# LinXueyuanStdio/LaTeX_OCR

Measured on NVIDIA H100. Metric: formula-images/sec (train step, 128x512 px, seq<=150), higher is better.
Workload: dtype bf16

## Files before the change

latex_ocr_b200/csrc/lo_common.cuh:

```cuda
#pragma once
#include <cuda_runtime.h>
#include <cuda_bf16.h>
#include <stdint.h>
#include <stdio.h>
#include <string.h>

#include "../../include/latex_ocr_b200.h"

typedef __nv_bfloat16 bf16;

namespace lo {

extern char g_err[512];
extern int64_t g_launches;

inline int fail(int code, const char* fmt, const char* a = "", long b = 0, long c = 0) {
  snprintf(g_err, sizeof(g_err), fmt, a, b, c);
  return code;
}

#define LO_CHECK_ARG(cond, what)                                                        \
  do {                                                                                  \
    if (!(cond)) return lo::fail(LO_EINVAL, "%s: invalid argument: " what " (line %ld)", __func__, __LINE__); \
  } while (0)

#define LO_CUDA(call)                                                                   \
  do {                                                                                  \
    cudaError_t e__ = (call);                                                           \
    if (e__ != cudaSuccess)                                                             \
      return lo::fail(LO_ECUDA, "%s: CUDA error %ld at line %ld", cudaGetErrorString(e__), (long)e__, __LINE__); \
  } while (0)

#define LO_LAUNCH_OK()                                                                  \
  do {                                                                                  \
    lo::g_launches++;                                                                   \
    cudaError_t e__ = cudaGetLastError();                                               \
    if (e__ != cudaSuccess)                                                             \
      return lo::fail(LO_ECUDA, "%s: launch failed (%ld) at line %ld", cudaGetErrorString(e__), (long)e__, __LINE__); \
  } while (0)

#define LO_TRY(call)                                                                    \
  do {                                                                                  \
    int r__ = (call);                                                                   \
    if (r__ != LO_OK) return r__;                                                       \
  } while (0)

inline int cdiv(long a, long b) { return (int)((a + b - 1) / b); }

constexpr int LO_NUM_SMS = 132;

#define LO_OPTIONS(X)                                                                                           \
  X(g_opt_att_pipe, "att_pipe", 1)                 \
  X(g_opt_pdl, "pdl", 1)                                                   \
  X(g_opt_att_abi_pdl, "att_abi_pdl", 0)             \
  X(g_opt_att_l2_keep_mb, "att_l2_keep_mb", 24)    \
  X(g_opt_att_nsplit, "att_nsplit", 0)                       \
  X(g_opt_att_cluster, "att_cluster", 1)                      \
  X(g_opt_att_maskbits, "att_maskbits", 1)                 \
  X(g_opt_att_bwd_mma, "att_bwd_mma", 1)                     \
  X(g_opt_dec_streams, "dec_streams", 1)             \
  X(g_opt_dec_fuse, "dec_fuse", 0)                                        \
  X(g_opt_dec_fuse_bwd, "dec_fuse_bwd", 0)                               \
  X(g_opt_dec_cl, "dec_cl", 0)                                                 \
  X(g_opt_dec_cl_bwd, "dec_cl_bwd", 0)                                        \
  X(g_opt_fuse_lstm, "fuse_lstm", 0)                               \
  X(g_opt_skinny_mma, "skinny_mma", 1)                               \
  X(g_opt_skinny_tma, "skinny_tma", 1)                                    \
  X(g_opt_skinny8, "skinny8", 1)                                        \
  X(g_opt_conv_persist, "conv_persist", 1)                      \
  X(g_opt_conv_mt2, "conv_mt2", 1)                            \
  X(g_opt_conv_mc, "conv_mc", 1)                                     \
  X(g_opt_wgrad256, "wgrad256", 0)                                   \
  X(g_opt_det, "deterministic", 0)                                             \
  X(g_opt_dbg_skip, "dbg_skip", 0)                                  \
  X(g_opt_l2_persist_mb, "l2_persist_mb", 0)

#define LO_OPTION_EXTERN(var, name, def) extern int var;
LO_OPTIONS(LO_OPTION_EXTERN)
#undef LO_OPTION_EXTERN

template <typename... KArgs, typename... Args>
inline cudaError_t launch_pdl(void (*kernel)(KArgs...), dim3 grid, dim3 block, size_t smem, cudaStream_t st, Args... args) {
  cudaLaunchConfig_t cfg{};
  cfg.gridDim = grid;
  cfg.blockDim = block;
  cfg.dynamicSmemBytes = smem;
  cfg.stream = st;
  cudaLaunchAttribute attr[1];
  attr[0].id = cudaLaunchAttributeProgrammaticStreamSerialization;
  attr[0].val.programmaticStreamSerializationAllowed = 1;
  cfg.attrs = attr;
  cfg.numAttrs = g_opt_pdl ? 1 : 0;
  return cudaLaunchKernelEx(&cfg, kernel, KArgs(args)...);
}
template <typename... KArgs, typename... Args>
inline cudaError_t launch_cluster(void (*kernel)(KArgs...), dim3 grid, dim3 block, size_t smem, cudaStream_t st, dim3 cl, bool pdl,
                                  Args... args) {
  cudaLaunchConfig_t cfg{};
  cfg.gridDim = grid;
  cfg.blockDim = block;
  cfg.dynamicSmemBytes = smem;
  cfg.stream = st;
  cudaLaunchAttribute attr[2];
  int n = 0;
  attr[n].id = cudaLaunchAttributeClusterDimension;
  attr[n].val.clusterDim.x = cl.x;
  attr[n].val.clusterDim.y = cl.y;
  attr[n].val.clusterDim.z = cl.z;
  n++;
  if (pdl && g_opt_pdl) {
    attr[n].id = cudaLaunchAttributeProgrammaticStreamSerialization;
    attr[n].val.programmaticStreamSerializationAllowed = 1;
    n++;
  }
  cfg.attrs = attr;
  cfg.numAttrs = n;
  return cudaLaunchKernelEx(&cfg, kernel, KArgs(args)...);
}

__device__ __forceinline__ float ldf(const float* p) { return *p; }
__device__ __forceinline__ float ldf(const bf16* p) { return __bfloat162float(*p); }
__device__ __forceinline__ void stf(float* p, float v) { *p = v; }
__device__ __forceinline__ void stf(bf16* p, float v) { *p = __float2bfloat16_rn(v); }
__device__ __forceinline__ float roundto(float v, const float*) { return v; }
__device__ __forceinline__ float roundto(float v, const bf16*) { return __bfloat162float(__float2bfloat16_rn(v)); }

__device__ __forceinline__ void ld8(const float* p, float* v) {
  float4 a = *reinterpret_cast<const float4*>(p);
  float4 b = *reinterpret_cast<const float4*>(p + 4);
  v[0] = a.x; v[1] = a.y; v[2] = a.z; v[3] = a.w; v[4] = b.x; v[5] = b.y; v[6] = b.z; v[7] = b.w;
}
__device__ __forceinline__ void ld8(const bf16* p, float* v) {
  uint4 u = *reinterpret_cast<const uint4*>(p);
  const uint32_t w[4] = {u.x, u.y, u.z, u.w};
#pragma unroll
  for (int i = 0; i < 4; i++) {
    v[2 * i] = __uint_as_float(w[i] << 16);
    v[2 * i + 1] = __uint_as_float(w[i] & 0xffff0000u);
  }
}
__device__ __forceinline__ void lds8(uint32_t saddr, float* v, const float*) {
  float4 a, b;
  asm volatile("ld.shared.v4.f32 {%0, %1, %2, %3}, [%4];" : "=f"(a.x), "=f"(a.y), "=f"(a.z), "=f"(a.w) : "r"(saddr));
  asm volatile("ld.shared.v4.f32 {%0, %1, %2, %3}, [%4];" : "=f"(b.x), "=f"(b.y), "=f"(b.z), "=f"(b.w) : "r"(saddr + 16));
  v[0] = a.x; v[1] = a.y; v[2] = a.z; v[3] = a.w; v[4] = b.x; v[5] = b.y; v[6] = b.z; v[7] = b.w;
}
__device__ __forceinline__ void lds8(uint32_t saddr, float* v, const bf16*) {
  uint32_t w[4];
  asm volatile("ld.shared.v4.b32 {%0, %1, %2, %3}, [%4];" : "=r"(w[0]), "=r"(w[1]), "=r"(w[2]), "=r"(w[3]) : "r"(saddr));
#pragma unroll
  for (int i = 0; i < 4; i++) {
    v[2 * i] = __uint_as_float(w[i] << 16);
    v[2 * i + 1] = __uint_as_float(w[i] & 0xffff0000u);
  }
}
__device__ __forceinline__ void st8(float* p, const float* v) {
  *reinterpret_cast<float4*>(p) = make_float4(v[0], v[1], v[2], v[3]);
  *reinterpret_cast<float4*>(p + 4) = make_float4(v[4], v[5], v[6], v[7]);
}
__device__ __forceinline__ void st8(bf16* p, const float* v) {
  uint32_t w[4];
#pragma unroll
  for (int i = 0; i < 4; i++) {
    __nv_bfloat162 h = __floats2bfloat162_rn(v[2 * i], v[2 * i + 1]);
    w[i] = *reinterpret_cast<uint32_t*>(&h);
  }
  *reinterpret_cast<uint4*>(p) = make_uint4(w[0], w[1], w[2], w[3]);
}

__device__ __forceinline__ float warp_sum(float v) {
#pragma unroll
  for (int o = 16; o > 0; o >>= 1) v += __shfl_xor_sync(0xffffffffu, v, o);
  return v;
}
__device__ __forceinline__ float warp_max(float v) {
#pragma unroll
  for (int o = 16; o > 0; o >>= 1) v = fmaxf(v, __shfl_xor_sync(0xffffffffu, v, o));
  return v;
}
__device__ __forceinline__ float sigmoidf_(float x) { return 1.0f / (1.0f + expf(-x)); }

__device__ __forceinline__ uint4 philox4x32_10(uint4 c, uint2 k) {
#pragma unroll
  for (int r = 0; r < 10; r++) {
    const uint32_t hi0 = __umulhi(0xD2511F53u, c.x), lo0 = 0xD2511F53u * c.x;
    const uint32_t hi1 = __umulhi(0xCD9E8D57u, c.z), lo1 = 0xCD9E8D57u * c.z;
    c = make_uint4(hi1 ^ c.y ^ k.x, lo1, hi0 ^ c.w ^ k.y, lo0);
    k.x += 0x9E3779B9u;
    k.y += 0xBB67AE85u;
  }
  return c;
}
__device__ __forceinline__ float u01(uint32_t x) { return (float)(x >> 8) * (1.0f / 16777216.0f); }
__device__ __forceinline__ float philox_dropout_mult(const unsigned long long* state, int b, int t, int j, float p, float scale) {
  const unsigned long long seed = state[0], call = state[1];
  const uint4 r = philox4x32_10(make_uint4((uint32_t)(j >> 2), (uint32_t)t, (uint32_t)b, (uint32_t)call),
                                make_uint2((uint32_t)seed, (uint32_t)(seed >> 32)));
  const uint32_t w = (j & 3) == 0 ? r.x : ((j & 3) == 1 ? r.y : ((j & 3) == 2 ? r.z : r.w));
  return u01(w) >= p ? scale : 0.f;
}

#define LO_DISPATCH_DT(dt, T, ...)                   \
  do {                                               \
    if ((dt) == LO_F32) { typedef float T; __VA_ARGS__; } \
    else if ((dt) == LO_BF16) { typedef bf16 T; __VA_ARGS__; } \
    else return lo::fail(LO_EINVAL, "%s: bad dtype %ld", __func__, (long)(dt)); \
  } while (0)

struct GemmDesc {
  int M, N, K;
  int64_t sam, sak, sbk, sbn, ldc;
  int batch;
  int64_t sA, sB, sC;
  const float* bias;
  int accumulate, relu;
};
int gemm(const void* A, int dtA, const void* B, int dtB, void* C, int dtC, const GemmDesc& d, int impl, cudaStream_t st);
int gemm_nt(const void* A, int dtA, int64_t lda, const void* W, int dtW, int64_t ldw, void* C, int dtC, int64_t ldc,
            int M, int N, int K, const float* bias, int accumulate, int relu, int impl, cudaStream_t st);
int gemm_tn(const void* A, int dtA, int64_t lda, const void* B, int dtB, int64_t ldb, void* C, int dtC, int64_t ldc,
            int M, int N, int K, int accumulate, int impl, cudaStream_t st);
int gemm_nn(const void* A, int dtA, int64_t lda, const void* B, int dtB, int64_t ldb, void* C, int dtC, int64_t ldc,
            int M, int N, int K, int accumulate, int impl, cudaStream_t st);
int colsum(const void* X, int dt, float* out, int M, int N, int64_t ld, int accumulate, cudaStream_t st);

struct AttFwdArgs {
  const void *att1, *enc;
  const float* att2; int64_t att2_stride;
  const float* wf;
  float* alpha; int64_t alpha_stride;
  float* ctx; float* gate_pre; int64_t gate_stride; float* gctx; bf16* gctx_bf;
  int B, R;
  void* work;
  int rows_per_img;
  int nsplit_hint;
  int act;
  int a_ch;
  uint8_t* mask_out;
  int abi = 0;
};
struct AttBwdArgs {
  const void *att1, *enc;
  const float *att2, *gate; int64_t o1_stride;
  const float* wf; const float* alpha; int64_t alpha_stride;
  const float* ctx; const float* dgctx; int64_t dg_stride;
  const float* dreg; int64_t dreg_stride; const float* sreg; int64_t sreg_stride;
  float* de; float* datt2; float* dgp; int64_t dcat_stride; bf16* datt2_bf; bf16* dgp_bf; float* dctx_out;
  int B, R;
  void* work;
  float* dwf_part;
  int nsplit_hint;
  int act;
  int a_ch;
  const uint8_t* mask_in;
  int abi = 0;
  void* datt1 = nullptr;
  int ordered_dwf = 0;
};
int attention_fwd_pipe(const AttFwdArgs& x, int dt, int C, cudaStream_t st);
int attention_bwd_pipe(const AttBwdArgs& x, int dt, int C, cudaStream_t st);
inline int64_t att_partials_offset(int B) { return B <= 1024 ? 4096 : ((int64_t)B * 4 + 255) / 256 * 256; }
struct AttRagged {
  const int32_t* reg_off;
  const int32_t* reg_off_host;
  void* map;
  int ctas;
};
int64_t attention_ragged_map_bytes(int B);
int attention_ragged_prepare(AttRagged& rg, int B, int rpi, cudaStream_t st);
int attention_fwd_ragged(const AttFwdArgs& x, const AttRagged& rg, int dt, int C, cudaStream_t st);

bool tc_available();
int tc_gemm_nt(const bf16* A, int64_t lda, const bf16* W, int64_t ldw, void* C, int dtC, int64_t ldc,
               int M, int N, int K, const float* bias, int accumulate, int relu, cudaStream_t st);
int tc_gemm_nt_ex(const bf16* A, int64_t lda, const bf16* W, int64_t ldw, void* C, int dtC, int64_t ldc, int M, int N, int K,
                  const float* bias, int accumulate, int relu, int splits, int atomic_acc, int small_n_tile, cudaStream_t st);
struct TcLstmEpi {
  const float* ptab; const int64_t* tok; int64_t tok_stride;
  const float* hh; int64_t hh_stride;
  const float* c_prev; float* gates; float* c_out; float* h_out; bf16* h_bf;
  float* hd; int64_t hd_stride; const float* dmask;
  int D, V;
  const unsigned long long* dstate; float dp; int row0, t_idx;
};
struct DecStepFwd {
  const bf16* gctx; int64_t ld_gctx;
  const bf16* wil; int64_t ld_wil;
  TcLstmEpi e;
  const bf16* wcat; int64_t ld_wcat;
  const float* bcat; float* o1_next; int64_t ld_o1; int N2;
  unsigned int* bar; unsigned int bar_target;
  int M, K;
};
int dec_step_fwd(const DecStepFwd& p, cudaStream_t st);
struct DecStepBwd {
  const bf16* dcat_a; int64_t ld_dcat;
  const bf16* wbwd2; int64_t ld_w2; int K2;
  int Ma;
  const float* dhd; int64_t dhd_stride; const float* dmask; const unsigned long long* dstate; float dp; int t_idx;
  float* dc; const float* gates; const float* c_prev; const float* c_cur;
  float* dG; bf16* dG_bf; int64_t dG_stride;
  const bf16* wbwd1; int64_t ld_w1; int K1;
  int Mb;
  float* dxh; int C, D;
  unsigned int* bar; unsigned int bar_target;
};
int dec_step_bwd(const DecStepBwd& p, cudaStream_t st);
bool dec_cl_fwd_ok(int D, int C, int N2);
bool dec_cl_bwd_ok(int D, int C, int A);
int dec_cl_fwd(const DecStepFwd& p, cudaStream_t st);
int dec_cl_bwd(const DecStepBwd& p, cudaStream_t st);
int cl_set_ts(long long* p);
int sk_set_ts(long long* p);
int tc_gemm_nt_lstm(const bf16* A, int64_t lda, const bf16* Wil, int64_t ldw, int M, int D, int K, const TcLstmEpi& e, cudaStream_t st);
int skinny_gemm_nt_lstm(const bf16* A, int64_t lda, const bf16* Wil, int64_t ldw, int M, int D, int K, const TcLstmEpi& e, cudaStream_t st);
int skinny_gemm_nt(const bf16* A, int64_t lda, const bf16* W, int64_t ldw, float* C, int64_t ldc, int M, int N, int K, const float* bias,
                   int splits, int atomic_acc, cudaStream_t st);
int tc_gemm_tn(const bf16* A, int64_t lda, const bf16* B, int64_t ldb, float* C, int64_t ldc, int M, int N, int K, cudaStream_t st);
int tc_gemm_tn_batched(const bf16* A, int64_t sAk, int64_t sAb, const bf16* B, int64_t sBk, int64_t sBb, float* C, int64_t ldc,
                       int64_t sCb, int M, int N, int K, int batch, cudaStream_t st);
int tc_conv3x3_wgrad(const bf16* x, const bf16* dy, float* dw, int N, int H, int W, int Cin, int Cout, int pad, cudaStream_t st);
int tc_conv3x3(const bf16* x, const bf16* w, const float* bias, const bf16* mask, bf16* y,
               int N, int H, int W, int Cin, int Cout, int pad, int relu, cudaStream_t st);

}
```

latex_ocr_b200/csrc/lo_tc.cu:

```cuda
#include <cuda.h>

#include <mutex>
#include <unordered_map>

#include "lo_common.cuh"
#include "lo_ptx.cuh"
#include "lo_wgmma.cuh"

namespace lo {

__device__ __forceinline__ void tma_load_2d(void* dst, const CUtensorMap* map, uint64_t* bar, int c0, int c1) {
  asm volatile("cp.async.bulk.tensor.2d.shared::cluster.global.mbarrier::complete_tx::bytes [%0], [%1, {%3, %4}], [%2];" ::"r"(
                   smem_u32(dst)),
               "l"(reinterpret_cast<uint64_t>(map)), "r"(smem_u32(bar)), "r"(c0), "r"(c1)
               : "memory");
}
__device__ __forceinline__ void tma_load_2d_hint(void* dst, const CUtensorMap* map, uint64_t* bar, int c0, int c1, uint64_t policy) {
  asm volatile(
      "cp.async.bulk.tensor.2d.shared::cluster.global.mbarrier::complete_tx::bytes.L2::cache_hint [%0], [%1, {%3, %4}], [%2], %5;" ::"r"(
          smem_u32(dst)),
      "l"(reinterpret_cast<uint64_t>(map)), "r"(smem_u32(bar)), "r"(c0), "r"(c1), "l"(policy)
      : "memory");
}
__device__ __forceinline__ void tma_load_3d(void* dst, const CUtensorMap* map, uint64_t* bar, int c0, int c1, int c2) {
// ... 286 lines not shown
          tc_store_pair(p, row_off + n0 + c, acc[4 * i + 2 * h] + s_bias[c], acc[4 * i + 2 * h + 1] + s_bias[c + 1], use_mask);
        }
      }
    }
    if (dbg && threadIdx.x == 0) p.dbg[6] = clock64();
  }
  if (MC) cluster_sync_all();
  if (dbg && threadIdx.x == 0) p.dbg[7] = clock64();
}

template <int NT, int STAGES, int MT>
struct TcPSmem {
  static constexpr int A_BYTES = TC_BM * TC_BK * 2;
  static constexpr int B_BYTES = NT * TC_BK * 2;
  static constexpr int STAGE_BYTES = MT * A_BYTES + B_BYTES;
  static constexpr int TOTAL = STAGES * STAGE_BYTES + 1024  + 256  + 2 * NT * 4 ;
};

template <int NT, int STAGES, int MT>
__global__ void __launch_bounds__(TC_THREADS, 1) tc_conv_p_kernel(const __grid_constant__ CUtensorMap mapA,
                                                                 const __grid_constant__ CUtensorMap mapB, TcParams p, int ntiles_n,
                                                                 int total_tiles, int mtiles) {
  using SM = TcPSmem<NT, STAGES, MT>;
  static_assert(MT * NT <= 256, "accumulator registers");
  extern __shared__ uint8_t smem_raw[];
  uint8_t* smem = reinterpret_cast<uint8_t*>((reinterpret_cast<uintptr_t>(smem_raw) + 1023) & ~(uintptr_t)1023);
  uint64_t* full_bar = reinterpret_cast<uint64_t*>(smem + STAGES * SM::STAGE_BYTES);
  uint64_t* empty_bar = full_bar + STAGES;
  float* s_bias = reinterpret_cast<float*>(smem + STAGES * SM::STAGE_BYTES + 256);

  const int warp = threadIdx.x >> 5, lane = threadIdx.x & 31;
  const int KB = p.K / TC_BK;
  const int cpb = p.Cin / TC_BK;
  const int per_img = p.tiles_w * p.tiles_h;

  if (warp == TC_CWARPS && lane == 0) {
    tma_prefetch_desc(&mapA);
    tma_prefetch_desc(&mapB);
    for (int s = 0; s < STAGES; s++) {
      mbar_init(full_bar + s, 2);
      mbar_init(empty_bar + s, TC_CWARPS);
    }
    fence_barrier_init();
  }
  pdl_wait();
  pdl_trigger();
  __syncthreads();

  if (warp == TC_CWARPS) {
    if (lane == 0) {
      uint32_t it = 0;
      for (int tile = blockIdx.x; tile < total_tiles; tile += gridDim.x) {
        const int mt0 = (tile / ntiles_n) * MT;
        const int nsub = min(MT, mtiles - mt0);
        int img[MT], h0[MT], w0[MT];
#pragma unroll
        for (int j = 0; j < MT; j++) {
          const int mt = min(mt0 + j, mtiles - 1);
          img[j] = mt / per_img;
          const int rem = mt % per_img;
          h0[j] = (rem / p.tiles_w) * p.BH;
          w0[j] = (rem % p.tiles_w) * p.BW;
        }
        for (int kb = 0; kb < KB; kb++, it++) {
          const int s = it % STAGES;
          const uint32_t ph = (it / STAGES) & 1;
          mbar_wait(empty_bar + s, ph ^ 1);
          mbar_expect_tx(full_bar + s, (uint32_t)nsub * SM::A_BYTES);
          const int tap = kb / cpb, cb = kb % cpb;
          const int r = tap / 3, q = tap % 3;
#pragma unroll
          for (int j = 0; j < MT; j++)
            if (j < nsub)
              tma_load_4d(smem + s * SM::STAGE_BYTES + j * SM::A_BYTES, &mapA, full_bar + s, cb * TC_BK, w0[j] + q - p.pad,
                          h0[j] + r - p.pad, img[j]);
        }
      }
    }
    __syncwarp();
  } else if (warp == TC_CWARPS + 1) {
    if (lane == 0) {
      const uint64_t polB = l2_policy_evict_last();
      uint32_t it = 0;
      for (int tile = blockIdx.x; tile < total_tiles; tile += gridDim.x) {
        const int n0 = (tile % ntiles_n) * NT;
        for (int kb = 0; kb < KB; kb++, it++) {
          const int s = it % STAGES;
          const uint32_t ph = (it / STAGES) & 1;
          mbar_wait(empty_bar + s, ph ^ 1);
          mbar_expect_tx(full_bar + s, SM::B_BYTES);
          tma_load_2d_hint(smem + s * SM::STAGE_BYTES + MT * SM::A_BYTES, &mapB, full_bar + s, kb * TC_BK, n0, polB);
        }
      }
    }
    __syncwarp();
  } else {
    const int wg = warp >> 2;
    const int rbase = wg * 64 + (warp & 3) * 16 + (lane >> 2);
    const int cq = 2 * (lane & 3);
    const bool use_mask = p.mask != nullptr;
    uint32_t it = 0, lt = 0;
    for (int tile = blockIdx.x; tile < total_tiles; tile += gridDim.x, lt++) {
      const int n0 = (tile % ntiles_n) * NT;
      const int mt0 = (tile / ntiles_n) * MT;
      const int nsub = min(MT, mtiles - mt0);
      float* sb = s_bias + (lt & 1) * NT;
      for (int c = threadIdx.x; c < NT; c += TC_CWARPS * 32) sb[c] = (p.bias && n0 + c < p.N) ? __ldg(p.bias + n0 + c) : 0.f;
      asm volatile("bar.sync 1, 256;" ::: "memory");
      float acc[MT][NT / 2];
      for (int kb = 0; kb < KB; kb++, it++) {
        const int s = it % STAGES;
        const uint32_t ph = (it / STAGES) & 1;
        mbar_wait(full_bar + s, ph);
        const uint32_t sa = smem_u32(smem + s * SM::STAGE_BYTES);
        wgmma_fence();
#pragma unroll
        for (int j = 0; j < MT; j++)
          tc_mma_kblock<NT>(acc[j], sa + j * SM::A_BYTES + wg * (SM::A_BYTES / 2), sa + MT * SM::A_BYTES, kb == 0);
        wgmma_commit();
        wgmma_wait0();
#pragma unroll
        for (int j = 0; j < MT; j++) wgmma_acc_fence<NT / 2>(acc[j]);
        __syncwarp();
        if (lane == 0) mbar_arrive(empty_bar + s);
      }
#pragma unroll
      for (int j = 0; j < MT; j++) {
        if (j >= nsub) continue;
        const int mt = mt0 + j;
        const int img = mt / per_img, rem = mt % per_img;
#pragma unroll
        for (int h = 0; h < 2; h++) {
          const int row = rbase + 8 * h;
          const int hh = (rem / p.tiles_w) * p.BH + row / p.BW, ww = (rem % p.tiles_w) * p.BW + row % p.BW;
          if (hh >= p.Ho || ww >= p.Wo) continue;
          const int64_t row_off = (((int64_t)img * p.Ho + hh) * p.Wo + ww) * p.ldc;
#pragma unroll
          for (int i = 0; i < NT / 8; i++) {
            if (n0 + 8 * i >= p.N) continue;
            const int c = 8 * i + cq;
            float f0 = acc[j][4 * i + 2 * h] + sb[c], f1 = acc[j][4 * i + 2 * h + 1] + sb[c + 1];
            if (p.relu) { f0 = fmaxf(f0, 0.f); f1 = fmaxf(f1, 0.f); }
            if (use_mask) {
              const uint32_t w = *reinterpret_cast<const uint32_t*>(p.mask + row_off + n0 + c);
              if (!(__uint_as_float(w << 16) > 0.f)) f0 = 0.f;
              if (!(__uint_as_float(w & 0xffff0000u) > 0.f)) f1 = 0.f;
            }
            __nv_bfloat162 hv = __floats2bfloat162_rn(f0, f1);
            *reinterpret_cast<__nv_bfloat162*>(reinterpret_cast<bf16*>(p.out) + row_off + n0 + c) = hv;
          }
        }
      }
    }
  }
}

__device__ __forceinline__ uint64_t make_mnmajor_sw128_desc(uint32_t saddr, uint32_t lbo_bytes) {
  uint64_t d = 0;
  d |= (uint64_t)((saddr & 0x3FFFF) >> 4);
  d |= (uint64_t)((lbo_bytes >> 4) & 0x3FFF) << 16;
  d |= (uint64_t)(1024 >> 4) << 32;
  d |= (uint64_t)1 << 62;
  return d;
}

struct WgParams {
  int Cin, Cout, Ho, Wo, pad;
  int BW, BH, tiles_w, tiles_h, kstages, per_split, ci_tiles;
  float* dw;
  int plain;
  int64_t ldc;
  int64_t batch_c;
  int ordered;
};

template <int NT, int STAGES>
__global__ void __launch_bounds__(TC_THREADS, 1) tc_wgrad_kernel(const __grid_constant__ CUtensorMap mapDY,
                                                                  const __grid_constant__ CUtensorMap mapX, WgParams p) {
  constexpr int BOX = 128 * 64 * 2;
  constexpr int A_BYTES = 2 * BOX, B_BYTES = (NT / 64) * BOX, STAGE_BYTES = A_BYTES + B_BYTES;
  extern __shared__ uint8_t smem_raw[];
  uint8_t* smem = reinterpret_cast<uint8_t*>((reinterpret_cast<uintptr_t>(smem_raw) + 1023) & ~(uintptr_t)1023);
  uint64_t* full_bar = reinterpret_cast<uint64_t*>(smem + STAGES * STAGE_BYTES);
  uint64_t* empty_bar = full_bar + STAGES;
  const int warp = threadIdx.x >> 5, lane = threadIdx.x & 31;
  const int co0 = (blockIdx.x / p.ci_tiles) * 128, ci0 = (blockIdx.x % p.ci_tiles) * NT;
  const int tap = p.plain == 2 ? 0 : blockIdx.y, r = tap / 3, q = tap % 3;
  const int bz = p.plain == 2 ? blockIdx.y : 0;
  const int ks0 = blockIdx.z * p.per_split;
  const int ks1 = min(p.kstages, ks0 + p.per_split);
  const int KS = ks1 - ks0;
  if (warp == TC_CWARPS && lane == 0) {
    tma_prefetch_desc(&mapDY);
    tma_prefetch_desc(&mapX);
    for (int s = 0; s < STAGES; s++) { mbar_init(full_bar + s, 2); mbar_init(empty_bar + s, TC_CWARPS); }
    fence_barrier_init();
  }
  __syncthreads();
  float acc[NT / 2];
  if (warp == TC_CWARPS) {
    if (lane == 0) {
      const int per_img = p.tiles_w * p.tiles_h;
      for (int i = 0; i < KS; i++) {
        const int s = i % STAGES;
        const uint32_t ph = (i / STAGES) & 1;
        mbar_wait(empty_bar + s, ph ^ 1);
        const int ks = ks0 + i;
        const int img = ks / per_img, rem = ks % per_img;
        const int h0 = (rem / p.tiles_w) * p.BH, w0 = (rem % p.tiles_w) * p.BW;
        uint8_t* sa = smem + s * STAGE_BYTES;
        mbar_expect_tx(full_bar + s, A_BYTES);
        if (p.plain == 2) {
          tma_load_3d(sa, &mapDY, full_bar + s, co0, ks * 128, bz);
          tma_load_3d(sa + BOX, &mapDY, full_bar + s, co0 + 64, ks * 128, bz);
        } else if (p.plain) {
          tma_load_2d(sa, &mapDY, full_bar + s, co0, ks * 128);
          tma_load_2d(sa + BOX, &mapDY, full_bar + s, co0 + 64, ks * 128);
        } else {
          tma_load_4d(sa, &mapDY, full_bar + s, co0, w0, h0, img);
          tma_load_4d(sa + BOX, &mapDY, full_bar + s, co0 + 64, w0, h0, img);
        }
      }
    }
    __syncwarp();
  } else if (warp == TC_CWARPS + 1) {
    if (lane == 0) {
      const int per_img = p.tiles_w * p.tiles_h;
      for (int i = 0; i < KS; i++) {
        const int s = i % STAGES;
        const uint32_t ph = (i / STAGES) & 1;
        mbar_wait(empty_bar + s, ph ^ 1);
        const int ks = ks0 + i;
        const int img = ks / per_img, rem = ks % per_img;
        const int h0 = (rem / p.tiles_w) * p.BH, w0 = (rem % p.tiles_w) * p.BW;
        uint8_t* sb = smem + s * STAGE_BYTES + A_BYTES;
        mbar_expect_tx(full_bar + s, B_BYTES);
        if (p.plain == 2) {
#pragma unroll
          for (int j = 0; j < NT / 64; j++) tma_load_3d(sb + j * BOX, &mapX, full_bar + s, ci0 + 64 * j, ks * 128, bz);
        } else if (p.plain) {
#pragma unroll
          for (int j = 0; j < NT / 64; j++) tma_load_2d(sb + j * BOX, &mapX, full_bar + s, ci0 + 64 * j, ks * 128);
        } else {
#pragma unroll
          for (int j = 0; j < NT / 64; j++)
            tma_load_4d(sb + j * BOX, &mapX, full_bar + s, ci0 + 64 * j, w0 + q - p.pad, h0 + r - p.pad, img);
        }
      }
    }
    __syncwarp();
  } else {
    const int wg = warp >> 2;
#pragma unroll
    for (int i = 0; i < NT / 2; i++) acc[i] = 0.f;
    for (int i = 0; i < KS; i++) {
      const int s = i % STAGES;
      const uint32_t ph = (i / STAGES) & 1;
      mbar_wait(full_bar + s, ph);
      const uint32_t sa = smem_u32(smem + s * STAGE_BYTES) + wg * BOX;
      const uint32_t sb = smem_u32(smem + s * STAGE_BYTES) + A_BYTES;
      wgmma_fence();
#pragma unroll
      for (int k = 0; k < 8; k++)
        Wgmma<NT, 1, 1>::mma(acc, make_mnmajor_sw128_desc(sa + k * 2048, BOX), make_mnmajor_sw128_desc(sb + k * 2048, BOX), 1u);
      wgmma_commit();
      wgmma_wait0();
      wgmma_acc_fence<NT / 2>(acc);
      __syncwarp();
      if (lane == 0) mbar_arrive(empty_bar + s);
    }
  }
  if (p.ordered && gridDim.z > 1) {
    float* part = reinterpret_cast<float*>(smem);
    if (warp < TC_CWARPS) {
      asm volatile("bar.sync 1, 256;" ::: "memory");
#pragma unroll
      for (int i = 0; i < NT / 2; i++) part[i * 256 + threadIdx.x] = acc[i];
    }
    cl_sync();
    if (cl_rank() == 0 && warp < TC_CWARPS) {
#pragma unroll
      for (int i = 0; i < NT / 2; i += 16) cl_sum_n<16>(part + i * 256 + threadIdx.x, 256, acc + i);
    }
    cl_sync();
    if (cl_rank() != 0) return;
  }
  if (warp < TC_CWARPS) {
    const int wg = warp >> 2, cq = 2 * (lane & 3);
#pragma unroll
    for (int h = 0; h < 2; h++) {
      const int co = co0 + wg * 64 + (warp & 3) * 16 + (lane >> 2) + 8 * h;
      if (co >= p.Cout) continue;
      float* orow = p.plain ? p.dw + (int64_t)bz * p.batch_c + (int64_t)co * p.ldc : p.dw + ((int64_t)co * 9 + tap) * p.Cin;
#pragma unroll
      for (int i = 0; i < NT / 8; i++) {
        const int ci = ci0 + 8 * i + cq;
        if (ci < p.Cin) atomicAdd(orow + ci, acc[4 * i + 2 * h]);
        if (ci + 1 < p.Cin) atomicAdd(orow + ci + 1, acc[4 * i + 2 * h + 1]);
      }
    }
  }
}

typedef CUresult (*PFN_tmapEncodeTiled)(CUtensorMap*, CUtensorMapDataType, cuuint32_t, void*, const cuuint64_t*, const cuuint64_t*,
                                        const cuuint32_t*, const cuuint32_t*, CUtensorMapInterleave, CUtensorMapSwizzle,
                                        CUtensorMapL2promotion, CUtensorMapFloatOOBfill);
static PFN_tmapEncodeTiled g_encode = nullptr;
static int g_tc_state = -1;

bool tc_available() {
  if (g_tc_state >= 0) return g_tc_state == 1;
  g_tc_state = 0;
  int dev = 0, major = 0;
  if (cudaGetDevice(&dev) != cudaSuccess) return false;
  if (cudaDeviceGetAttribute(&major, cudaDevAttrComputeCapabilityMajor, dev) != cudaSuccess || major != 9) return false;
  void* fn = nullptr;
  cudaDriverEntryPointQueryResult qres;
  if (cudaGetDriverEntryPoint("cuTensorMapEncodeTiled", &fn, cudaEnableDefault, &qres) != cudaSuccess || fn == nullptr ||
      qres != cudaDriverEntryPointSuccess)
    return false;
  g_encode = (PFN_tmapEncodeTiled)fn;
  g_tc_state = 1;
  return true;
}

struct MapKey {
  const void* base; int rank; cuuint64_t dims[4]; cuuint64_t str[3]; cuuint32_t box[4];
  bool operator==(const MapKey& o) const { return memcmp(this, &o, sizeof(MapKey)) == 0; }
};
struct MapKeyHash {
  size_t operator()(const MapKey& k) const {
    const uint64_t* w = reinterpret_cast<const uint64_t*>(&k);
    uint64_t h = 1469598103934665603ull;
    for (size_t i = 0; i < sizeof(MapKey) / 8; i++) { h ^= w[i]; h *= 1099511628211ull; }
    return (size_t)h;
  }
};
static std::unordered_map<MapKey, CUtensorMap, MapKeyHash> g_map_cache;
static std::mutex g_map_mutex;

static int make_map(CUtensorMap* m, const void* base, int rank, const cuuint64_t* dims, const cuuint64_t* strides_bytes,
                    const cuuint32_t* box) {
  MapKey key;
  memset(&key, 0, sizeof(key));
  key.base = base; key.rank = rank;
  for (int i = 0; i < rank; i++) { key.dims[i] = dims[i]; key.box[i] = box[i]; }
  for (int i = 0; i + 1 < rank; i++) key.str[i] = strides_bytes[i];
  {
    std::lock_guard<std::mutex> lk(g_map_mutex);
    auto it = g_map_cache.find(key);
    if (it != g_map_cache.end()) { *m = it->second; return LO_OK; }
  }
  cuuint32_t estr[4] = {1, 1, 1, 1};
  CUresult r = g_encode(m, CU_TENSOR_MAP_DATA_TYPE_BFLOAT16, (cuuint32_t)rank, const_cast<void*>(base), dims, strides_bytes, box, estr,
                        CU_TENSOR_MAP_INTERLEAVE_NONE, CU_TENSOR_MAP_SWIZZLE_128B, CU_TENSOR_MAP_L2_PROMOTION_L2_256B,
                        CU_TENSOR_MAP_FLOAT_OOB_FILL_NONE);
  if (r != CUDA_SUCCESS) return fail(LO_ECUDA, "%s: cuTensorMapEncodeTiled failed (%ld)", "tc", (long)r);
  std::lock_guard<std::mutex> lk(g_map_mutex);
  if (g_map_cache.size() > 20000) g_map_cache.clear();
  g_map_cache.emplace(key, *m);
  return LO_OK;
}

long long* g_tc_dbg = nullptr;

template <int NT, int STAGES, int MC>
static int launch_tc(const CUtensorMap& mA, const CUtensorMap& mB, const TcParams& p, int mtiles, int splits, cudaStream_t st) {
  using SM = TcSmem<NT, STAGES>;
  static bool attr_set = false;
  if (!attr_set) {
    LO_CUDA(cudaFuncSetAttribute(tc_gemm_conv_kernel<NT, STAGES, MC>, cudaFuncAttributeMaxDynamicSharedMemorySize, SM::TOTAL));
    attr_set = true;
  }
  dim3 grid(cdiv(p.N, NT), mtiles, splits);
  cudaLaunchConfig_t cfg{};
  cfg.gridDim = grid;
  cfg.blockDim = dim3(TC_THREADS);
  cfg.dynamicSmemBytes = SM::TOTAL;
  cfg.stream = st;
  cudaLaunchAttribute attr[2];
  int n = 0;
  if (g_opt_pdl) {
    attr[n].id = cudaLaunchAttributeProgrammaticStreamSerialization;
    attr[n].val.programmaticStreamSerializationAllowed = 1;
    n++;
  }
  if (MC) {
    attr[n].id = cudaLaunchAttributeClusterDimension;
    attr[n].val.clusterDim.x = 2;
    attr[n].val.clusterDim.y = 1;
    attr[n].val.clusterDim.z = 1;
    n++;
  }
  cfg.attrs = attr;
  cfg.numAttrs = n;
  LO_CUDA(cudaLaunchKernelEx(&cfg, tc_gemm_conv_kernel<NT, STAGES, MC>, mA, mB, p));
  LO_LAUNCH_OK();
  return LO_OK;
}

static int launch_tc_any(const CUtensorMap& mA, const CUtensorMap& mB, TcParams& p, int mtiles, int splits, int nt, cudaStream_t st,
                         int mc = 0) {
  const int KB = p.K / TC_BK;
  if (splits < 1) splits = 1;
  if (splits > KB) splits = KB;
  p.kb_per_split = cdiv(KB, splits);
  splits = cdiv(KB, p.kb_per_split);
  p.atomic = splits > 1 ? 1 : p.atomic;
  if (nt == 64 && mtiles == 1 && p.kb_per_split > 4 && g_opt_skinny8) return launch_tc<64, 8, 0>(mA, mB, p, mtiles, splits, st);
  if (nt == 64) return launch_tc<64, 4, 0>(mA, mB, p, mtiles, splits, st);
  if (mc) return launch_tc<128, 3, 1>(mA, mB, p, mtiles, splits, st);
  return launch_tc<128, 3, 0>(mA, mB, p, mtiles, splits, st);
}

static TcLstmEpi g_lstm_epi;
static bool g_lstm_epi_on = false;

int tc_gemm_nt_ex(const bf16* A, int64_t lda, const bf16* W, int64_t ldw, void* C, int dtC, int64_t ldc, int M, int N, int K,
                  const float* bias, int accumulate, int relu, int splits, int atomic_acc, int small_n_tile, cudaStream_t st) {
  if (!tc_available()) return fail(LO_ENOTSUP, "%s: needs an sm_90 device", __func__);
  LO_CHECK_ARG(K % 64 == 0 && lda % 8 == 0 && ldw % 8 == 0 && ldc % 8 == 0 && ldc >= (N + 7) / 8 * 8, "K%64, ld%8, ldc >= roundup8(N)");
  LO_CHECK_ARG(((uintptr_t)A & 15) == 0 && ((uintptr_t)W & 15) == 0 && ((uintptr_t)C & 15) == 0, "16-byte alignment");
  CUtensorMap mA, mB;
  const int NT = (N <= 64 || small_n_tile) ? 64 : 128;
  const int mc = (g_opt_conv_mc && NT == 128 && cdiv(N, 128) % 2 == 0 && splits <= 1 && !atomic_acc) ? 1 : 0;
  {
    cuuint64_t dims[2] = {(cuuint64_t)K, (cuuint64_t)M};
    cuuint64_t str[1] = {(cuuint64_t)lda * 2};
    cuuint32_t box[2] = {64, (cuuint32_t)(mc ? 64 : 128)};
    LO_TRY(make_map(&mA, A, 2, dims, str, box));
  }
  {
    cuuint64_t dims[2] = {(cuuint64_t)K, (cuuint64_t)N};
    cuuint64_t str[1] = {(cuuint64_t)ldw * 2};
    cuuint32_t box[2] = {64, (cuuint32_t)NT};
    LO_TRY(make_map(&mB, W, 2, dims, str, box));
  }
  LO_CHECK_ARG(!(splits > 1 || atomic_acc) || (dtC == LO_F32 && !relu), "split-K needs fp32 output without ReLU");
  TcParams p{};
  p.M = M; p.N = N; p.K = K; p.conv = 0;
  p.bias = bias; p.mask = nullptr; p.out = C; p.ldc = ldc;
  p.out_f32 = (dtC == LO_F32); p.accumulate = accumulate; p.relu = relu; p.atomic = atomic_acc;
  p.w_evict_last = (M <= 128) ? 1 : 0;
  p.dbg = g_tc_dbg;
  if (g_lstm_epi_on) {
    const TcLstmEpi& e = g_lstm_epi;
    p.lstm = 1;
    p.l_ptab = e.ptab; p.l_tok = e.tok; p.l_tok_stride = e.tok_stride; p.l_hh = e.hh; p.l_hh_stride = e.hh_stride;
    p.l_cprev = e.c_prev; p.l_gates = e.gates; p.l_c = e.c_out; p.l_h = e.h_out; p.l_hbf = e.h_bf;
    p.l_hd = e.hd; p.l_hd_stride = e.hd_stride; p.l_dmask = e.dmask; p.l_D = e.D; p.l_V = e.V;
  }
  return launch_tc_any(mA, mB, p, cdiv(M, TC_BM), splits, NT, st, mc);
}

int tc_gemm_nt_lstm(const bf16* A, int64_t lda, const bf16* Wil, int64_t ldw, int M, int D, int K, const TcLstmEpi& e, cudaStream_t st) {
  g_lstm_epi = e;
  g_lstm_epi_on = true;
  const int r = tc_gemm_nt_ex(A, lda, Wil, ldw, e.gates , LO_F32, 4 * D, M, 4 * D, K, nullptr, 0, 0, 1, 0, 1, st);
  g_lstm_epi_on = false;
  return r;
}

int tc_gemm_nt(const bf16* A, int64_t lda, const bf16* W, int64_t ldw, void* C, int dtC, int64_t ldc, int M, int N, int K,
               const float* bias, int accumulate, int relu, cudaStream_t st) {
  return tc_gemm_nt_ex(A, lda, W, ldw, C, dtC, ldc, M, N, K, bias, accumulate, relu, 1, 0, 0, st);
}

template <int NT, int STAGES, int MT>
static int launch_conv_p(const CUtensorMap& mA, const CUtensorMap& mB, const TcParams& p, int mtiles, cudaStream_t st) {
  using SM = TcPSmem<NT, STAGES, MT>;
  static bool attr_set = false;
  static int n_sm = 0;
  if (!attr_set) {
    LO_CUDA(cudaFuncSetAttribute(tc_conv_p_kernel<NT, STAGES, MT>, cudaFuncAttributeMaxDynamicSharedMemorySize, SM::TOTAL));
    int dev = 0;
    LO_CUDA(cudaGetDevice(&dev));
    LO_CUDA(cudaDeviceGetAttribute(&n_sm, cudaDevAttrMultiProcessorCount, dev));
    attr_set = true;
  }
  const int ntn = cdiv(p.N, NT);
  const int total = cdiv(mtiles, MT) * ntn;
  const int grid = total < n_sm ? total : n_sm;
  LO_CUDA(launch_pdl(tc_conv_p_kernel<NT, STAGES, MT>, dim3(grid), dim3(TC_THREADS), (size_t)SM::TOTAL, st, mA, mB, p, ntn, total, mtiles));
  LO_LAUNCH_OK();
  return LO_OK;
}

int tc_conv3x3(const bf16* x, const bf16* w, const float* bias, const bf16* mask, bf16* y, int N, int H, int W, int Cin, int Cout,
               int pad, int relu, cudaStream_t st) {
  if (!tc_available()) return fail(LO_ENOTSUP, "%s: needs an sm_90 device", __func__);
  LO_CHECK_ARG(Cin % 64 == 0 && Cout % 8 == 0, "Cin%64==0, Cout%8==0");
  const int Ho = H + 2 * pad - 2, Wo = W + 2 * pad - 2;
  int BW = 128;
  while (BW > 8 && BW / 2 >= Wo) BW /= 2;
  const int BH = 128 / BW;
  if (g_opt_conv_persist) {
    const int NTp = Cout % 256 == 0 ? 256 : (Cout > 64 ? 128 : 64);
    CUtensorMap mA, mB;
    {
      cuuint64_t dims[4] = {(cuuint64_t)Cin, (cuuint64_t)W, (cuuint64_t)H, (cuuint64_t)N};
      cuuint64_t str[3] = {(cuuint64_t)Cin * 2, (cuuint64_t)W * Cin * 2, (cuuint64_t)H * W * Cin * 2};
      cuuint32_t box[4] = {64, (cuuint32_t)BW, (cuuint32_t)BH, 1};
      LO_TRY(make_map(&mA, x, 4, dims, str, box));
    }
    {
      cuuint64_t dims[2] = {(cuuint64_t)9 * Cin, (cuuint64_t)Cout};
      cuuint64_t str[1] = {(cuuint64_t)9 * Cin * 2};
      cuuint32_t box[2] = {64, (cuuint32_t)NTp};
      LO_TRY(make_map(&mB, w, 2, dims, str, box));
    }
    TcParams p{};
    p.M = N * Ho * Wo; p.N = Cout; p.K = 9 * Cin; p.conv = 1;
    p.Ho = Ho; p.Wo = Wo; p.Cin = Cin; p.pad = pad;
    p.BW = BW; p.BH = BH; p.tiles_w = cdiv(Wo, BW); p.tiles_h = cdiv(Ho, BH);
    p.bias = bias; p.mask = mask; p.out = y; p.ldc = Cout; p.relu = relu;
    const int mtiles = N * p.tiles_w * p.tiles_h;
    if (NTp == 256) return launch_conv_p<256, 4, 1>(mA, mB, p, mtiles, st);
    if (NTp == 128) return g_opt_conv_mt2 ? launch_conv_p<128, 4, 2>(mA, mB, p, mtiles, st) : launch_conv_p<128, 6, 1>(mA, mB, p, mtiles, st);
    return g_opt_conv_mt2 ? launch_conv_p<64, 4, 2>(mA, mB, p, mtiles, st) : launch_conv_p<64, 8, 1>(mA, mB, p, mtiles, st);
  }
  CUtensorMap mA, mB;
  const int NT = Cout <= 64 ? 64 : 128;
  const int mc = (g_opt_conv_mc && NT == 128 && cdiv(Cout, 128) % 2 == 0) ? 1 : 0;
  const int hbw = mc ? (BH >= 2 ? BW : BW / 2) : BW, hbh = mc ? (BH >= 2 ? BH / 2 : 1) : BH;
  {
    cuuint64_t dims[4] = {(cuuint64_t)Cin, (cuuint64_t)W, (cuuint64_t)H, (cuuint64_t)N};
    cuuint64_t str[3] = {(cuuint64_t)Cin * 2, (cuuint64_t)W * Cin * 2, (cuuint64_t)H * W * Cin * 2};
    cuuint32_t box[4] = {64, (cuuint32_t)hbw, (cuuint32_t)hbh, 1};
    LO_TRY(make_map(&mA, x, 4, dims, str, box));
  }
  {
    cuuint64_t dims[2] = {(cuuint64_t)9 * Cin, (cuuint64_t)Cout};
    cuuint64_t str[1] = {(cuuint64_t)9 * Cin * 2};
    cuuint32_t box[2] = {64, (cuuint32_t)NT};
    LO_TRY(make_map(&mB, w, 2, dims, str, box));
  }
  TcParams p{};
  p.M = N * Ho * Wo; p.N = Cout; p.K = 9 * Cin; p.conv = 1;
  p.Ho = Ho; p.Wo = Wo; p.Cin = Cin; p.pad = pad;
  p.BW = BW; p.BH = BH; p.tiles_w = cdiv(Wo, BW); p.tiles_h = cdiv(Ho, BH);
  p.bias = bias; p.mask = mask; p.out = y; p.ldc = Cout;
  p.out_f32 = 0; p.accumulate = 0; p.relu = relu;
  p.dbg = g_tc_dbg;
  p.half_w = (mc && BH < 2) ? BW / 2 : 0;
  p.half_h = (mc && BH >= 2) ? BH / 2 : 0;
  const int mtiles = N * p.tiles_w * p.tiles_h;
  LO_CHECK_ARG(mtiles <= 65535, "too many M tiles for grid.y");
  return launch_tc_any(mA, mB, p, mtiles, 1, NT, st, mc);
}


template <int NT, int STAGES>
static int launch_wgrad(const CUtensorMap& mDY, const CUtensorMap& mX, const WgParams& p, dim3 grid, cudaStream_t st) {
  constexpr int TOTAL = STAGES * (2 + NT / 64) * 16384 + 1024 + 256;
  static bool attr_set = false;
  if (!attr_set) {
    LO_CUDA(cudaFuncSetAttribute(tc_wgrad_kernel<NT, STAGES>, cudaFuncAttributeMaxDynamicSharedMemorySize, TOTAL));
    attr_set = true;
  }
  if (p.ordered)
    LO_CUDA(launch_cluster(tc_wgrad_kernel<NT, STAGES>, grid, dim3(TC_THREADS), (size_t)TOTAL, st, dim3(1, 1, grid.z), false, mDY, mX, p));
  else
    tc_wgrad_kernel<NT, STAGES><<<grid, TC_THREADS, TOTAL, st>>>(mDY, mX, p);
  LO_LAUNCH_OK();
  return LO_OK;
}

int tc_conv3x3_wgrad(const bf16* x, const bf16* dy, float* dw, int N, int H, int W, int Cin, int Cout, int pad, cudaStream_t st) {
  if (!tc_available()) return fail(LO_ENOTSUP, "%s: needs an sm_90 device", __func__);
  LO_CHECK_ARG(Cin % 64 == 0 && Cout % 128 == 0, "Cin%64==0, Cout%128==0");
  const int Ho = H + 2 * pad - 2, Wo = W + 2 * pad - 2;
  int BW = 128;
  while (BW > 8 && BW / 2 >= Wo) BW /= 2;
  const int BH = 128 / BW;
  CUtensorMap mDY, mX;
  {
    cuuint64_t dims[4] = {(cuuint64_t)Cout, (cuuint64_t)Wo, (cuuint64_t)Ho, (cuuint64_t)N};
    cuuint64_t str[3] = {(cuuint64_t)Cout * 2, (cuuint64_t)Wo * Cout * 2, (cuuint64_t)Ho * Wo * Cout * 2};
    cuuint32_t box[4] = {64, (cuuint32_t)BW, (cuuint32_t)BH, 1};
    LO_TRY(make_map(&mDY, dy, 4, dims, str, box));
  }
  {
    cuuint64_t dims[4] = {(cuuint64_t)Cin, (cuuint64_t)W, (cuuint64_t)H, (cuuint64_t)N};
    cuuint64_t str[3] = {(cuuint64_t)Cin * 2, (cuuint64_t)W * Cin * 2, (cuuint64_t)H * W * Cin * 2};
    cuuint32_t box[4] = {64, (cuuint32_t)BW, (cuuint32_t)BH, 1};
    LO_TRY(make_map(&mX, x, 4, dims, str, box));
  }
  WgParams p{};
  p.Cin = Cin; p.Cout = Cout; p.Ho = Ho; p.Wo = Wo; p.pad = pad;
  p.BW = BW; p.BH = BH; p.tiles_w = cdiv(Wo, BW); p.tiles_h = cdiv(Ho, BH);
  p.kstages = N * p.tiles_w * p.tiles_h;
  p.dw = dw;
  const int NT = (g_opt_wgrad256 && Cin % 256 == 0) ? 256 : (Cin >= 128 ? 128 : 64);
  p.ci_tiles = Cin / NT;
  const int tiles = (Cout / 128) * p.ci_tiles * 9;
  int splits = cdiv(NT == 256 ? LO_NUM_SMS : LO_NUM_SMS * 2, tiles);
  if (g_opt_det && splits > 8) splits = 8;
  if (splits > p.kstages) splits = p.kstages;
  if (splits < 1) splits = 1;
  p.per_split = cdiv(p.kstages, splits);
  splits = cdiv(p.kstages, p.per_split);
  p.ordered = g_opt_det && splits > 1;
  dim3 grid((Cout / 128) * p.ci_tiles, 9, splits);
  if (NT == 256) return launch_wgrad<256, 2>(mDY, mX, p, grid, st);
  if (NT == 128) return launch_wgrad<128, 3>(mDY, mX, p, grid, st);
  return launch_wgrad<64, 4>(mDY, mX, p, grid, st);
}

int tc_gemm_tn(const bf16* A, int64_t lda, const bf16* B, int64_t ldb, float* C, int64_t ldc, int M, int N, int K, cudaStream_t st) {
  if (!tc_available()) return fail(LO_ENOTSUP, "%s: needs an sm_90 device", __func__);
  LO_CHECK_ARG(lda % 8 == 0 && ldb % 8 == 0, "lda%8, ldb%8");
  LO_CHECK_ARG(((uintptr_t)A & 15) == 0 && ((uintptr_t)B & 15) == 0, "16-byte alignment");
  CUtensorMap mA, mB;
  {
    cuuint64_t dims[2] = {(cuuint64_t)M, (cuuint64_t)K};
    cuuint64_t str[1] = {(cuuint64_t)lda * 2};
    cuuint32_t box[2] = {64, 128};
    LO_TRY(make_map(&mA, A, 2, dims, str, box));
  }
  {
    cuuint64_t dims[2] = {(cuuint64_t)N, (cuuint64_t)K};
    cuuint64_t str[1] = {(cuuint64_t)ldb * 2};
    cuuint32_t box[2] = {64, 128};
    LO_TRY(make_map(&mB, B, 2, dims, str, box));
  }
  WgParams p{};
  p.plain = 1; p.Cout = M; p.Cin = N; p.dw = C; p.ldc = ldc;
  p.tiles_w = p.tiles_h = 1; p.BW = 128; p.BH = 1;
  p.kstages = cdiv(K, 128);
  const int NT = N > 64 ? 128 : 64;
  p.ci_tiles = cdiv(N, NT);
  const int mt = cdiv(M, 128);
  const int tiles = mt * p.ci_tiles;
  int splits = cdiv(LO_NUM_SMS * 2, tiles);
  if (g_opt_det && splits > 8) splits = 8;
  if (splits > p.kstages) splits = p.kstages;
  if (splits < 1) splits = 1;
  p.per_split = cdiv(p.kstages, splits);
  splits = cdiv(p.kstages, p.per_split);
  p.ordered = g_opt_det && splits > 1;
  dim3 grid(mt * p.ci_tiles, 1, splits);
  if (NT == 128) return launch_wgrad<128, 3>(mA, mB, p, grid, st);
  return launch_wgrad<64, 4>(mA, mB, p, grid, st);
}

int tc_gemm_tn_batched(const bf16* A, int64_t sAk, int64_t sAb, const bf16* B, int64_t sBk, int64_t sBb, float* C, int64_t ldc,
                       int64_t sCb, int M, int N, int K, int batch, cudaStream_t st) {
  if (!tc_available()) return fail(LO_ENOTSUP, "%s: needs an sm_90 device", __func__);
  LO_CHECK_ARG(sAk % 8 == 0 && sAb % 8 == 0 && sBk % 8 == 0 && sBb % 8 == 0, "strides must be multiples of 8 elements");
  LO_CHECK_ARG(((uintptr_t)A & 15) == 0 && ((uintptr_t)B & 15) == 0 && batch >= 1 && batch <= 65535, "alignment / batch");
  CUtensorMap mA, mB;
  {
    cuuint64_t dims[3] = {(cuuint64_t)M, (cuuint64_t)K, (cuuint64_t)batch};
    cuuint64_t str[2] = {(cuuint64_t)sAk * 2, (cuuint64_t)sAb * 2};
    cuuint32_t box[3] = {64, 128, 1};
    LO_TRY(make_map(&mA, A, 3, dims, str, box));
  }
  {
    cuuint64_t dims[3] = {(cuuint64_t)N, (cuuint64_t)K, (cuuint64_t)batch};
    cuuint64_t str[2] = {(cuuint64_t)sBk * 2, (cuuint64_t)sBb * 2};
    cuuint32_t box[3] = {64, 128, 1};
    LO_TRY(make_map(&mB, B, 3, dims, str, box));
  }
  WgParams p{};
  p.plain = 2; p.Cout = M; p.Cin = N; p.dw = C; p.ldc = ldc; p.batch_c = sCb;
  p.tiles_w = p.tiles_h = 1; p.BW = 128; p.BH = 1;
  p.kstages = cdiv(K, 128);
  p.per_split = p.kstages;
  const int NT = N > 64 ? 128 : 64;
  p.ci_tiles = cdiv(N, NT);
  dim3 grid(cdiv(M, 128) * p.ci_tiles, batch, 1);
  if (NT == 128) return launch_wgrad<128, 3>(mA, mB, p, grid, st);
  return launch_wgrad<64, 4>(mA, mB, p, grid, st);
}

}
```

Baseline: 2453.

## Add sliding-window conv3x3 wgrad kernel reusing input rows across taps

Adds a new weight-gradient kernel for narrow feature maps. Each CTA handles one tap column across all three tap rows. It keeps a ring of single-row input tiles in shared memory, so overlapping rows are loaded once and reused by three consumer warpgroups, instead of reloading a full input box for each of the nine taps. A separate cost model picks the split count. This cuts TMA traffic and redundant loads, at the price of a more complex barrier ring, more shared memory, and changed grid occupancy.

```diff
diff --git a/latex_ocr_b200/csrc/lo_common.cuh b/latex_ocr_b200/csrc/lo_common.cuh
--- a/latex_ocr_b200/csrc/lo_common.cuh
+++ b/latex_ocr_b200/csrc/lo_common.cuh
@@ -71,6 +71,7 @@
   X(g_opt_conv_mt2, "conv_mt2", 1)                            \
   X(g_opt_conv_mc, "conv_mc", 1)                                     \
   X(g_opt_wgrad256, "wgrad256", 0)                                   \
+  X(g_opt_wgrad_win, "wgrad_win", 1)               \
   X(g_opt_det, "deterministic", 0)                                             \
   X(g_opt_dbg_skip, "dbg_skip", 0)                                  \
   X(g_opt_l2_persist_mb, "l2_persist_mb", 0)
diff --git a/latex_ocr_b200/csrc/lo_tc.cu b/latex_ocr_b200/csrc/lo_tc.cu
--- a/latex_ocr_b200/csrc/lo_tc.cu
+++ b/latex_ocr_b200/csrc/lo_tc.cu
@@ -612,6 +612,136 @@
   }
 }
 
+constexpr int WIN_CWARPS = 12;
+constexpr int WIN_THREADS = (WIN_CWARPS + 2) * 32;
+constexpr int WIN_BOX = 128 * 64 * 2;
+constexpr int WIN_DY_STAGES = 3, WIN_RING = 5;
+constexpr int WIN_X_BYTES = WIN_RING * 2 * WIN_BOX;
+constexpr int WIN_MAX_SLOTS = 40;
+constexpr int WIN_SMEM = WIN_DY_STAGES * WIN_BOX + WIN_X_BYTES + 1024  + 1024 ;
+
+__global__ void __launch_bounds__(WIN_THREADS, 1) tc_wgrad_win_kernel(const __grid_constant__ CUtensorMap mapDY,
+                                                                       const __grid_constant__ CUtensorMap mapX, WgParams p) {
+  extern __shared__ uint8_t smem_raw[];
+  uint8_t* smem = reinterpret_cast<uint8_t*>((reinterpret_cast<uintptr_t>(smem_raw) + 1023) & ~(uintptr_t)1023);
+  uint8_t* xs = smem + WIN_DY_STAGES * WIN_BOX;
+  uint64_t* dy_full = reinterpret_cast<uint64_t*>(xs + WIN_X_BYTES);
+  uint64_t* dy_empty = dy_full + WIN_DY_STAGES;
+  uint64_t* x_full = dy_empty + WIN_DY_STAGES;
+  uint64_t* x_empty = x_full + WIN_MAX_SLOTS;
+  const int warp = threadIdx.x >> 5, lane = threadIdx.x & 31;
+  const int co0 = (blockIdx.x / p.ci_tiles) * 64, ci0 = (blockIdx.x % p.ci_tiles) * 128;
+  const int q = blockIdx.y;
+  const int ks0 = blockIdx.z * p.per_split;
+  const int KS = min(p.kstages, ks0 + p.per_split) - ks0;
+  const int ring = WIN_RING * p.BH, win = p.BH + 2;
+  const int box_bytes = p.BW * 128, row_bytes = 2 * box_bytes;
+  if (warp == WIN_CWARPS && lane == 0) {
+    tma_prefetch_desc(&mapDY);
+    tma_prefetch_desc(&mapX);
+    for (int s = 0; s < WIN_DY_STAGES; s++) { mbar_init(dy_full + s, 1); mbar_init(dy_empty + s, WIN_CWARPS); }
+    for (int s = 0; s < ring; s++) { mbar_init(x_full + s, 1); mbar_init(x_empty + s, WIN_CWARPS); }
+    fence_barrier_init();
+  }
+  __syncthreads();
+  if (warp == WIN_CWARPS) {
+    if (lane == 0) {
+      for (int i = 0; i < KS; i++) {
+        const int s = i % WIN_DY_STAGES;
+        mbar_wait(dy_empty + s, ((i / WIN_DY_STAGES) & 1) ^ 1);
+        const int ks = ks0 + i;
+        mbar_expect_tx(dy_full + s, WIN_BOX);
+        tma_load_4d(smem + s * WIN_BOX, &mapDY, dy_full + s, co0, 0, (ks % p.tiles_h) * p.BH, ks / p.tiles_h);
+      }
+    }
+    __syncwarp();
+  } else if (warp == WIN_CWARPS + 1) {
+    if (lane == 0) {
+      int slot = 0;
+      uint32_t ph = 0;
+      for (int i = 0; i < KS; i++) {
+        const int ks = ks0 + i;
+        const int img = ks / p.tiles_h, h0 = (ks % p.tiles_h) * p.BH;
+        for (int t = (i == 0 || h0 == 0) ? 0 : 2; t < win; t++) {
+          mbar_wait(x_empty + slot, ph ^ 1);
+          mbar_expect_tx(x_full + slot, row_bytes);
+          tma_load_4d(xs + slot * row_bytes, &mapX, x_full + slot, ci0, q - p.pad, h0 + t - p.pad, img);
+          tma_load_4d(xs + slot * row_bytes + box_bytes, &mapX, x_full + slot, ci0 + 64, q - p.pad, h0 + t - p.pad, img);
+          if (++slot == ring) { slot = 0; ph ^= 1; }
+        }
+      }
+    }
+    __syncwarp();
+  } else {
+    const int r = warp >> 2;
+    const uint32_t xs_u32 = smem_u32(xs);
+    const int lbw = 31 - __clz(p.BW);
+    float acc[64];
+#pragma unroll
+    for (int i = 0; i < 64; i++) acc[i] = 0.f;
+    int base = 0;
+    uint32_t bph = 0;
+    for (int i = 0; i < KS; i++) {
+      const int s = i % WIN_DY_STAGES;
+      mbar_wait(dy_full + s, (i / WIN_DY_STAGES) & 1);
+      for (int t = 0; t < win; t++) {
+        const int sl = base + t;
+        if (sl >= ring) mbar_wait(x_full + sl - ring, bph ^ 1); else mbar_wait(x_full + sl, bph);
+      }
+      const uint32_t sa = smem_u32(smem + s * WIN_BOX);
+      wgmma_fence();
+#pragma unroll
+      for (int k = 0; k < 8; k++) {
+        int sl = base + ((16 * k) >> lbw) + r;
+        if (sl >= ring) sl -= ring;
+        const uint32_t off = (uint32_t)((16 * k) & (p.BW - 1)) * 128;
+        Wgmma<128, 1, 1>::mma(acc, make_mnmajor_sw128_desc(sa + k * 2048, WIN_BOX),
+                              make_mnmajor_sw128_desc(xs_u32 + sl * row_bytes + off, box_bytes), 1u);
+      }
+      wgmma_commit();
+      wgmma_wait0();
+      wgmma_acc_fence<64>(acc);
+      __syncwarp();
+      const int nrel = (i == KS - 1 || (ks0 + i + 1) % p.tiles_h == 0) ? win : p.BH;
+      if (lane == 0) {
+        mbar_arrive(dy_empty + s);
+        for (int t = 0; t < nrel; t++) {
+          const int sl = base + t;
+          mbar_arrive(x_empty + (sl >= ring ? sl - ring : sl));
+        }
+      }
+      base += nrel;
+      if (base >= ring) { base -= ring; bph ^= 1; }
+    }
+    if (p.ordered && gridDim.z > 1) {
+      float* part = reinterpret_cast<float*>(smem);
+      asm volatile("bar.sync 1, 384;" ::: "memory");
+#pragma unroll
+      for (int i = 0; i < 64; i++) part[i * 384 + threadIdx.x] = acc[i];
+      cl_sync();
+      if (cl_rank() == 0) {
+#pragma unroll
+        for (int i = 0; i < 64; i += 16) cl_sum_n<16>(part + i * 384 + threadIdx.x, 384, acc + i);
+      }
+      cl_sync();
+      if (cl_rank() != 0) return;
+    }
+    const int cq = 2 * (lane & 3);
+#pragma unroll
+    for (int h = 0; h < 2; h++) {
+      const int co = co0 + (warp & 3) * 16 + (lane >> 2) + 8 * h;
+      float* orow = p.dw + ((int64_t)co * 9 + 3 * r + q) * p.Cin + ci0 + cq;
+#pragma unroll
+      for (int i = 0; i < 16; i++) {
+        atomicAdd(orow + 8 * i, acc[4 * i + 2 * h]);
+        atomicAdd(orow + 8 * i + 1, acc[4 * i + 2 * h + 1]);
+      }
+    }
+    return;
+  }
+  if (p.ordered && gridDim.z > 1) { cl_sync(); cl_sync(); }
+}
+
 typedef CUresult (*PFN_tmapEncodeTiled)(CUtensorMap*, CUtensorMapDataType, cuuint32_t, void*, const cuuint64_t*, const cuuint64_t*,
                                         const cuuint32_t*, const cuuint32_t*, CUtensorMapInterleave, CUtensorMapSwizzle,
                                         CUtensorMapL2promotion, CUtensorMapFloatOOBfill);
@@ -876,6 +1006,30 @@
   return LO_OK;
 }
 
+static int launch_wgrad_win(const CUtensorMap& mDY, const CUtensorMap& mX, const WgParams& p, dim3 grid, cudaStream_t st) {
+  static bool attr_set = false;
+  if (!attr_set) {
+    LO_CUDA(cudaFuncSetAttribute(tc_wgrad_win_kernel, cudaFuncAttributeMaxDynamicSharedMemorySize, WIN_SMEM));
+    attr_set = true;
+  }
+  if (p.ordered)
+    LO_CUDA(launch_cluster(tc_wgrad_win_kernel, grid, dim3(WIN_THREADS), (size_t)WIN_SMEM, st, dim3(1, 1, grid.z), false, mDY, mX, p));
+  else
+    tc_wgrad_win_kernel<<<grid, WIN_THREADS, WIN_SMEM, st>>>(mDY, mX, p);
+  LO_LAUNCH_OK();
+  return LO_OK;
+}
+
+static int wgrad_win_splits(int ctas_per_split, int kstages) {
+  int best = 1;
+  long best_cost = 0;
+  for (int s = 1; s <= 16 && s <= kstages; s++) {
+    const long cost = (long)cdiv(ctas_per_split * s, LO_NUM_SMS) * (cdiv(kstages, s) + 8);
+    if (s == 1 || cost < best_cost) { best = s; best_cost = cost; }
+  }
+  return best;
+}
+
 int tc_conv3x3_wgrad(const bf16* x, const bf16* dy, float* dw, int N, int H, int W, int Cin, int Cout, int pad, cudaStream_t st) {
   if (!tc_available()) return fail(LO_ENOTSUP, "%s: needs an sm_90 device", __func__);
   LO_CHECK_ARG(Cin % 64 == 0 && Cout % 128 == 0, "Cin%64==0, Cout%128==0");
@@ -883,6 +1037,8 @@
   int BW = 128;
   while (BW > 8 && BW / 2 >= Wo) BW /= 2;
   const int BH = 128 / BW;
+  const int NT = (g_opt_wgrad256 && Cin % 256 == 0) ? 256 : (Cin >= 128 ? 128 : 64);
+  const bool win = g_opt_wgrad_win && NT != 256 && Cin % 128 == 0 && Wo <= BW && BW >= 16;
   CUtensorMap mDY, mX;
   {
     cuuint64_t dims[4] = {(cuuint64_t)Cout, (cuuint64_t)Wo, (cuuint64_t)Ho, (cuuint64_t)N};
@@ -893,7 +1049,7 @@
   {
     cuuint64_t dims[4] = {(cuuint64_t)Cin, (cuuint64_t)W, (cuuint64_t)H, (cuuint64_t)N};
     cuuint64_t str[3] = {(cuuint64_t)Cin * 2, (cuuint64_t)W * Cin * 2, (cuuint64_t)H * W * Cin * 2};
-    cuuint32_t box[4] = {64, (cuuint32_t)BW, (cuuint32_t)BH, 1};
+    cuuint32_t box[4] = {64, (cuuint32_t)BW, (cuuint32_t)(win ? 1 : BH), 1};
     LO_TRY(make_map(&mX, x, 4, dims, str, box));
   }
   WgParams p{};
@@ -901,7 +1057,6 @@
   p.BW = BW; p.BH = BH; p.tiles_w = cdiv(Wo, BW); p.tiles_h = cdiv(Ho, BH);
   p.kstages = N * p.tiles_w * p.tiles_h;
   p.dw = dw;
-  const int NT = (g_opt_wgrad256 && Cin % 256 == 0) ? 256 : (Cin >= 128 ? 128 : 64);
   p.ci_tiles = Cin / NT;
   const int tiles = (Cout / 128) * p.ci_tiles * 9;
   int splits = cdiv(NT == 256 ? LO_NUM_SMS : LO_NUM_SMS * 2, tiles);
@@ -911,6 +1066,15 @@
   p.per_split = cdiv(p.kstages, splits);
   splits = cdiv(p.kstages, p.per_split);
   p.ordered = g_opt_det && splits > 1;
+  if (win) {
+    p.ci_tiles = Cin / 128;
+    const int wtiles = (Cout / 64) * p.ci_tiles;
+    if (!g_opt_det) {
+      p.per_split = cdiv(p.kstages, wgrad_win_splits(3 * wtiles, p.kstages));
+      splits = cdiv(p.kstages, p.per_split);
+    }
+    return launch_wgrad_win(mDY, mX, p, dim3(wtiles, 3, splits), st);
+  }
   dim3 grid((Cout / 128) * p.ci_tiles, 9, splits);
   if (NT == 256) return launch_wgrad<256, 2>(mDY, mX, p, grid, st);
   if (NT == 128) return launch_wgrad<128, 3>(mDY, mX, p, grid, st);
```

Result: no change. 2468 (median of 6 runs) (+0.6%).
